# artpixls/ART

Measured on AMD Instinct MI355X. Metric: megapixels/sec end-to-end (AMaZE+FTblockDN+tone), 45 MP Bayer, higher is better.
Workload: dtype f32; 1 GPU; AMaZE + getImage/matrix + ImProcFunctions::denoise (chroma noise-curve map, FTblockDN wavelet shrinkage luma 40 / chroma 15 / gamma 1.7 + DCT detail recovery 50) + exposure 0.3 EV + tone curve STD, 8192x5464 Bayer RGGB fp32, 1 frame per GPU per step (BASELINE configs[2]); frame=8192x5464, lanes_per_gpu=1, parallelism=frame-per-gpu x1, completion_records=1, completion_via=single process

## Files before the change

art_amd/csrc/api_internal.h:

```cpp
#pragma once
#include <hip/hip_runtime.h>
#include <dlfcn.h>
#include <cmath>
#include <cstdio>
#include <cstdarg>
#include <cstring>
#include <new>
#include <string>
#include <thread>
#include <vector>
#include <algorithm>

#include "../../include/artgpu.h"
#include "kernels.h"
#include "dehaze.h"
#include "textureboost.h"
#include "colorcorrection.h"
#include "smoothing.h"
#include "toneequalizer.h"
#include "filmsim.h"
#include "masks.h"
#include "sharpen.h"

struct artgpu_ctx {
    int device = 0;
    hipStream_t stream = nullptr;
    hipStream_t aux = nullptr;
    hipEvent_t aux_ev[2] = {nullptr, nullptr};
    hipStream_t dn_stream[1] = {nullptr};
    hipEvent_t dn_ev[2] = {nullptr, nullptr};
    const float *gam_tab = nullptr; float gam_key[6] = {};
    struct Shared {
        int opt_sharpen_fused = 1;
        int opt_te_group_thread = 0;
        int opt_te_fuse_upsample = 1;
        int opt_lut_lds = 1;
        int opt_dn_streams = 0;
        int opt_dn_fused = 1;
        int opt_dn_detail_plain = 0;
        int opt_dn_mad_fold = 1;
        int opt_dn_mad_fold_grid = 0;
        int opt_dn_debug_stall = -1;
        long opt_dn_wait_ms = 0;
        int opt_io_direct = -1;
        int opt_cu_reserve = 0;
        int opt_amaze_path = 0;
        int opt_amaze_split = 0;
        long opt_amaze_zero_mask = 0x81f0;
        int opt_amaze_zero_frame = 16;
        int opt_amaze_poison = -1;
        int opt_roctx = 0;
        int opt_amaze_overlap = 1;
        int opt_amaze_grid = 0;
        int opt_rcd_rows = 8;
        int curve_tail_kind = ARTGPU_CURVE_TAIL_HOST;
        double curve_tail_y = 1.0;
        artgpu::ParamCurve curve_tail_pc = {};
        artgpu_progress_fn progress_fn = nullptr;
        void *progress_user = nullptr;
        const artgpu_mask_params *pipe_lc = nullptr, *pipe_tb = nullptr;
        int pipe_nlc = 0, pipe_ntb = 0;
        const artgpu_color_correction_region *pipe_cc = nullptr;
        const artgpu_mask_params *pipe_cc_masks = nullptr;
        int pipe_ncc = 0;
        const artgpu_smoothing_region *pipe_sm = nullptr;
        const artgpu_mask_params *pipe_sm_masks = nullptr;
        int pipe_nsm = 0;
        int pipe_te_on = 0;
        artgpu_tone_equalizer_params pipe_te = {};
        const artgpu_clut *pipe_fs = nullptr;
        artgpu_film_simulation_params pipe_fs_par = {};
        int pipe_fs_after = 0;
    } shared;
    float *sh_host = nullptr;
    hipEvent_t sh_ev = nullptr;
    struct PipeMasks { std::vector<artgpu_mask_params> m; std::vector<std::vector<double>> curves; std::vector<artgpu_plane> areas; } pipe_lc_own, pipe_tb_own;
    template <typename Region> struct PipeRegions { std::vector<Region> regs; std::vector<artgpu_plane> planes; PipeMasks masks; };
    PipeRegions<artgpu_color_correction_region> pipe_cc_own;
    PipeRegions<artgpu_smoothing_region> pipe_sm_own;
    artgpu_clut *pipe_fs_own = nullptr;
    std::string err;
    int *fs_diag = nullptr;
    long long batch_px = 0;
    const int *dn_fold_flags = nullptr; int dn_fold_ranges[8][2] = {}; int dn_fold_nranges = 0;
    int dn_form = -1, dn_form_streak = 0;
    float *arena = nullptr;
    size_t arena_bytes = 0;
    static constexpr int NSTAGE = 8;
    float *stage[NSTAGE] = {};
    size_t stage_bytes[NSTAGE] = {};
    static constexpr int NPOOL = 96;
    float *pool[NPOOL] = {};
// ... 222 lines not shown
```

art_amd/csrc/artgpu_api.hip:

```cpp
#include "api_internal.h"

using namespace artgpu;
using namespace artgpu::api;

namespace {

int const_table_dev(artgpu_ctx *ctx, int slot, size_t nfloats, void (*fill)(float *), const char *what, float **out)
{
    const bool fresh = ctx->pool[slot] == nullptr;
    const int rc = pool_get(ctx, slot, nfloats * 4, out);
    if (rc || !fresh) return rc;
    std::vector<float> host(nfloats);
    fill(host.data());
    hipError_t e = hipMemcpyAsync(*out, host.data(), nfloats * 4, hipMemcpyHostToDevice, ctx->stream);
    if (e == hipSuccess) e = hipStreamSynchronize(ctx->stream);
    if (e != hipSuccess) {
        (void)hipFree(ctx->pool[slot]); ctx->pool[slot] = nullptr; ctx->pool_bytes[slot] = 0;
        *out = nullptr;
        return fail(ctx, ARTGPU_EHIP, "upload of the %s failed: %s", what, hipGetErrorString(e));
    }
    return ARTGPU_OK;
}

void build_lab_tabs(float *host)
// ... 312 lines not shown
    HIPCHK(ctx, hipSetDevice(ctx->device));
    hipEvent_t ev = nullptr;
    if (hipEventCreateWithFlags(&ev, hipEventDisableTiming) == hipSuccess) {
        if (hipEventRecord(ev, ctx->stream) == hipSuccess) (void)hipStreamWaitEvent(next, ev, 0);
        (void)hipEventDestroy(ev);
    }
    (void)hipGetLastError();
    ctx->stream = next;
    return ARTGPU_OK;
}

int artgpu_synchronize(artgpu_ctx *ctx)
{
    if (!ctx) return ARTGPU_EINVAL;
    HIPCHK(ctx, hipSetDevice(ctx->device));
    HIPCHK(ctx, hipStreamSynchronize(ctx->stream));
    return check_async_faults(ctx);
}

int artgpu_set_curve_tail(artgpu_ctx *ctx, int kind, double y_last)
{
    if (!ctx) return ARTGPU_EINVAL;
    if (kind < ARTGPU_CURVE_TAIL_LUT || kind > ARTGPU_CURVE_TAIL_HOST) return fail(ctx, ARTGPU_EINVAL, "set_curve_tail: kind %d (a parametric curve: artgpu_set_curve_tail_parametric)", kind);
    ctx->shared.curve_tail_kind = kind;
    ctx->shared.curve_tail_y = y_last;
    return ARTGPU_OK;
}

int artgpu_set_curve_tail_parametric(artgpu_ctx *ctx, const double *p, int np)
{
    if (!ctx) return ARTGPU_EINVAL;
    if (!p || (np != 8 && np != 9)) return fail(ctx, ARTGPU_EINVAL, "set_curve_tail_parametric: 8 or 9 parameters (p[0] = DCT_Parametric)");
    if (p[4] == 0.0 && p[5] == 0.0 && p[6] == 0.0 && p[7] == 0.0) return fail(ctx, ARTGPU_EINVAL, "set_curve_tail_parametric: an identity curve has no Curve object (ARTGPU_CURVE_TAIL_LUT)");
    pc_init(ctx->shared.curve_tail_pc, p, np);
    ctx->shared.curve_tail_kind = ARTGPU_CURVE_TAIL_PARAMETRIC;
    return ARTGPU_OK;
}

int artgpu_get_option(artgpu_ctx *ctx, const char *name, long *value)
{
    if (!ctx || !name || !value) return ARTGPU_EINVAL;
    const std::string n(name);
    if (n.rfind("amaze_counter", 0) == 0 && n.size() == 14 && n[13] >= '0' && n[13] <= '7') {
        if (!ctx->amz_lists || ctx->amz_nstream <= 0) { *value = 0; return ARTGPU_OK; }
        HIPCHK(ctx, hipSetDevice(ctx->device));
        HIPCHK(ctx, hipStreamSynchronize(ctx->stream));
        const size_t nfixed = (((size_t)ctx->amz_nstream + (1 + ctx->amz_narena) + (1 + ctx->amz_narena + ctx->amz_nstream) + 3) / 4) * 4;
        int v = 0;
        HIPCHK(ctx, hipMemcpy(&v, reinterpret_cast<int *>(ctx->amz_lists) + nfixed + 4 + 2 * (size_t)ctx->amz_nstream + (n[13] - '0'), sizeof(int), hipMemcpyDeviceToHost));
        *value = v;
        return ARTGPU_OK;
    }
    if (n == "dn_mad_fold") { *value = ctx->shared.opt_dn_mad_fold; return ARTGPU_OK; }
    if (n == "cu_reserve") { *value = ctx->shared.opt_cu_reserve; return ARTGPU_OK; }
    if (n == "io_direct") { *value = ctx->shared.opt_io_direct; return ARTGPU_OK; }
    if (n == "te_group_thread") { *value = ctx->shared.opt_te_group_thread; return ARTGPU_OK; }
    if (n == "te_fuse_upsample") { *value = ctx->shared.opt_te_fuse_upsample; return ARTGPU_OK; }
    if (n.rfind("dn_mad_bits", 0) == 0 && n.size() > 11) {
        const int k = std::atoi(n.c_str() + 11);
        if (k < 0 || k > 95 || !ctx->dn_fold_flags) return fail(ctx, ARTGPU_EINVAL, "get_option: %s: word 0 .. 95 of a context that has denoised", name);
        HIPCHK(ctx, hipSetDevice(ctx->device));
        HIPCHK(ctx, hipStreamSynchronize(ctx->stream));
        int v = 0;
        HIPCHK(ctx, hipMemcpy(&v, ctx->dn_fold_flags - 96 + k, sizeof v, hipMemcpyDeviceToHost));
        *value = v;
        return ARTGPU_OK;
    }
    if (n == "dn_mad_fold_settled" || n == "dn_mad_fold_fallback") {
        HIPCHK(ctx, hipSetDevice(ctx->device));
        HIPCHK(ctx, hipStreamSynchronize(ctx->stream));
        int flags[96] = {};
        if (ctx->dn_fold_nranges) HIPCHK(ctx, hipMemcpy(flags, ctx->dn_fold_flags, sizeof flags, hipMemcpyDeviceToHost));
        const int want = n == "dn_mad_fold_settled" ? 1 : 2;
        long cnt = 0;
        for (int r = 0; r < ctx->dn_fold_nranges; ++r)
            for (int k = 0; k < ctx->dn_fold_ranges[r][1]; ++k) cnt += flags[ctx->dn_fold_ranges[r][0] + k] == want;
        *value = cnt;
        return ARTGPU_OK;
    }
    return fail(ctx, ARTGPU_EINVAL, "get_option: unknown option '%s'", name);
}

int artgpu_set_option(artgpu_ctx *ctx, const char *name, long value)
{
    if (!ctx || !name) return ARTGPU_EINVAL;
    const std::string n(name);
    if (n == "amaze_path") { if (value < 0 || value > 1) return fail(ctx, ARTGPU_EINVAL, "amaze_path: 0 or 1"); ctx->shared.opt_amaze_path = (int)value; }
    else if (n == "amaze_split") ctx->shared.opt_amaze_split = value != 0;
    else if (n == "amaze_overlap") ctx->shared.opt_amaze_overlap = value != 0;
    else if (n == "amaze_grid") { if (value < 0) return fail(ctx, ARTGPU_EINVAL, "amaze_grid: >= 0"); ctx->shared.opt_amaze_grid = (int)value; }
    else if (n == "amaze_zero_mask") ctx->shared.opt_amaze_zero_mask = value;
    else if (n == "amaze_zero_frame") ctx->shared.opt_amaze_zero_frame = (int)value;
    else if (n == "amaze_poison") ctx->shared.opt_amaze_poison = (int)value;
    else if (n == "roctx") ctx->shared.opt_roctx = value != 0;
    else if (n == "dn_streams") ctx->shared.opt_dn_streams = value != 0;
    else if (n == "dn_fused") ctx->shared.opt_dn_fused = (int)value;
    else if (n == "dn_mad_fold") ctx->shared.opt_dn_mad_fold = value != 0;
    else if (n == "dn_mad_fold_grid") { if (value < 0 || value > 65536) return fail(ctx, ARTGPU_EINVAL, "dn_mad_fold_grid: 0 (default) .. 65536 workgroups"); ctx->shared.opt_dn_mad_fold_grid = (int)value; }
    else if (n == "dn_detail_plain") { if (value < 0 || value > 3) return fail(ctx, ARTGPU_EINVAL, "dn_detail_plain: 0 .. 3"); ctx->shared.opt_dn_detail_plain = (int)value; }
    else if (n == "dn_debug_stall") ctx->shared.opt_dn_debug_stall = (int)value;
    else if (n == "dn_wait_ms") ctx->shared.opt_dn_wait_ms = value < 0 ? 0 : value;
    else if (n == "lut_lds") ctx->shared.opt_lut_lds = value != 0;
    else if (n == "te_group_thread") ctx->shared.opt_te_group_thread = value != 0;
    else if (n == "te_fuse_upsample") ctx->shared.opt_te_fuse_upsample = value != 0;
    else if (n == "sharpen_fused") ctx->shared.opt_sharpen_fused = value != 0;
    else if (n == "cu_reserve") { if (value < 0 || value > 4096) return fail(ctx, ARTGPU_EINVAL, "cu_reserve: 0 .. 4096"); ctx->shared.opt_cu_reserve = (int)value; }
    else if (n == "io_direct") { if (value < -1 || value > 4096) return fail(ctx, ARTGPU_EINVAL, "io_direct: -1 (automatic), 0 .. 4096 workgroups"); ctx->shared.opt_io_direct = (int)value; }
    else if (n == "rcd_rows") { if (value != 4 && value != 8) return fail(ctx, ARTGPU_EINVAL, "rcd_rows: 4 or 8"); ctx->shared.opt_rcd_rows = (int)value; }
    else return fail(ctx, ARTGPU_EINVAL, "set_option: unknown option '%s'", name);
    return ARTGPU_OK;
}

int artgpu_set_progress_callback(artgpu_ctx *ctx, artgpu_progress_fn fn, void *user)
{
    if (!ctx) return ARTGPU_EINVAL;
    ctx->shared.progress_fn = fn;
    ctx->shared.progress_user = user;
    return ARTGPU_OK;
}

int artgpu_enable_timing(artgpu_ctx *ctx, int enable)
{
    if (!ctx) return ARTGPU_EINVAL;
    ctx->timing = enable != 0;
    return ARTGPU_OK;
}

int artgpu_get_timings(const artgpu_ctx *ctx, artgpu_timings *out)
{
    if (!ctx || !out) return ARTGPU_EINVAL;
    *out = ctx->last;
    return ARTGPU_OK;
}

size_t artgpu_scratch_bytes(const artgpu_ctx *ctx)
{
    if (!ctx) return 0;
    size_t s = ctx->arena_bytes;
    for (int k = 0; k < artgpu_ctx::NSTAGE; ++k) s += ctx->stage_bytes[k];
    s += ctx->lut_bytes;
    for (int k = 0; k < artgpu_ctx::NPOOL; ++k) s += ctx->pool_bytes[k];
    return s;
}

int artgpu_trim_scratch(artgpu_ctx *ctx)
{
    if (!ctx) return ARTGPU_EINVAL;
    HIPCHK(ctx, hipSetDevice(ctx->device));
    HIPCHK(ctx, hipStreamSynchronize(ctx->stream));
    if (ctx->aux) HIPCHK(ctx, hipStreamSynchronize(ctx->aux));
    if (ctx->dn_stream[0]) HIPCHK(ctx, hipStreamSynchronize(ctx->dn_stream[0]));
    if (ctx->amz_side) HIPCHK(ctx, hipStreamSynchronize(ctx->amz_side));
// ... 349 lines not shown

}

namespace {

struct DnFusion {
    float pre_scale, post_scale;
    GetImageFuse gi;
    int exp_on;
    float exp_scale, exp_black;
    int tail_on;
    float tail_scale, tail_black;
    int ccalc_nonneg;
};

void build_dct_tabs(float *host)
{
    float *tm_in = host, *tm_out = tm_in + 4096, *ct = tm_out + 4096, *ctt = ct + 4096;
    const float epsilon = 0.001f / (64 * 64);
    const int border = 4;
    for (int i = 0; i < 64; ++i) {
        const float i1 = std::abs((i > 32 ? i - 64 + 1 : i));
        const float vmask = (i1 < border ? (float)0 + (std::sin((M_PI * i1) / (2 * border)) * std::sin((M_PI * i1) / (2 * border))) : 1.0f);
        const float vmask2 = (i1 < 2 * border ? (std::sin((M_PI * i1) / (2 * border)) * std::sin((M_PI * i1) / (2 * border))) : 1.0f);
        for (int j = 0; j < 64; ++j) {
            const float j1 = std::abs((j > 32 ? j - 64 + 1 : j));
            const double sj = std::sin((M_PI * j1) / (2 * border));
            tm_in[i * 64 + j] = (vmask * (j1 < border ? sj * sj : 1.0f)) + epsilon;
            tm_out[i * 64 + j] = (vmask2 * (j1 < 2 * border ? sj * sj : 1.0f)) + epsilon;
            ct[i * 64 + j] = (float)std::cos(M_PI * (j + 0.5) * i / 64.0);
            ctt[j * 64 + i] = ct[i * 64 + j];
        }
    }
}

struct DnPlan {
    int w, h, w2, h2;
    size_t n, n2;
    bool lab_mode, do_detail, useNoiseCCurve;
    float noisevarL;
    bool denoiseLuminance;
    float gam, gamthresh, gamslope, igam, igamthresh, igamslope, gain;
    float realred, realblue, noisevarab_r, noisevarab_b, maxNoiseVarab;
    bool aggressive, autoch;
    int levwav, nsub;
    bool too_small;
    int rad[10], maxrad;
    bool fork;
    bool mad_fold;
    int fold_g0, fold_g1;
    bool fused, merged, merged_mad;
    bool two_chroma;
    int detail_plain;
    long long wait_ticks;
    int stall_band, stall_strip;
};

DnPlan dn_plan(int w, int h, const artgpu_denoise_params *p, double scale, double expcomp, uint32_t flags, bool want_resid, bool has_ccalc,
               int opt_dn_streams, int opt_dn_fused, int opt_dn_detail_plain, long opt_dn_wait_ms, int opt_dn_debug_stall, int opt_dn_mad_fold, int opt_dn_mad_fold_grid)
{
    DnPlan pl = {};
    const int w2 = (w + 1) / 2, h2 = (h + 1) / 2;
    pl.w = w; pl.h = h; pl.w2 = w2; pl.h2 = h2; pl.n = (size_t)w * h; pl.n2 = (size_t)w2 * h2;
    pl.lab_mode = p->color_space == 1;
    pl.do_detail = !(flags & ARTGPU_DN_SKIP_DETAIL_RECOVERY);
    pl.useNoiseCCurve = has_ccalc;
    pl.detail_plain = opt_dn_detail_plain == 1 ? 3 : opt_dn_detail_plain == 2 ? 1 : opt_dn_detail_plain == 3 ? 2 : 0;
    pl.wait_ticks = (long long)opt_dn_wait_ms * 100000LL;
    pl.stall_band = opt_dn_debug_stall < 0 ? -1 : opt_dn_debug_stall >> 16;
    pl.stall_strip = opt_dn_debug_stall < 0 ? -1 : opt_dn_debug_stall & 0xffff;

    const float noiseluma = (float)p->luminance;
    const double nl_t = (noiseluma / 125.0) * (1.0 + noiseluma / 25.0);
    const float noisevarL = (float)(nl_t * nl_t);
    const bool denoiseLuminance = noisevarL > 0.00001f;
    const float gam = (float)p->gamma;
    const float gamthresh = 0.001f;
    const float gamslope = (float)(std::exp(std::log((double)gamthresh) / gam) / gamthresh);
    pl.noisevarL = noisevarL; pl.denoiseLuminance = denoiseLuminance;
    pl.gam = gam; pl.gamthresh = gamthresh; pl.gamslope = gamslope;
    pl.igam = 1.f / gam; pl.igamthresh = gamthresh * gamslope; pl.igamslope = 1.f / gamslope;
    pl.gain = std::pow(2.0f, float(expcomp));
    const float interm_med = (float)p->chrominance / 10.0;
    float intermred = p->chrominance_red_green > 0. ? (p->chrominance_red_green / 10.) : (float)p->chrominance_red_green / 7.0;
    float intermblue = p->chrominance_blue_yellow > 0. ? (p->chrominance_blue_yellow / 10.) : (float)p->chrominance_blue_yellow / 7.0;
    float realred = interm_med + intermred;
    if (realred <= 0.f) realred = 0.001f;
    float realblue = interm_med + intermblue;
    if (realblue <= 0.f) realblue = 0.001f;
    const float noisevarab_r = realred * realred, noisevarab_b = realblue * realblue;
    pl.realred = realred; pl.realblue = realblue; pl.noisevarab_r = noisevarab_r; pl.noisevarab_b = noisevarab_b;
    pl.maxNoiseVarab = noisevarab_b > noisevarab_r ? noisevarab_b : noisevarab_r;
    int levwav = 5;
    const float maxreal = realred > realblue ? realred : realblue;
    if (maxreal < 8.f) levwav = 5; else if (maxreal < 10.f) levwav = 6; else if (maxreal < 15.f) levwav = 7; else levwav = 8;
    const bool aggressive = p->aggressive != 0;
    if (aggressive) levwav += 2;
    if (levwav > 8) levwav = 8;
    { const int t = int(levwav - std::ceil(std::log(scale))); levwav = t > 5 ? t : 5; }
    const int minsizetile = w < h ? w : h;
    int maxlev2 = 8;
    if (minsizetile < 256) maxlev2 = 7;
    if (minsizetile < 128) maxlev2 = 6;
    if (minsizetile < 64) maxlev2 = 5;
    if (minsizetile < 32) maxlev2 = 4;
    if (minsizetile < 16) maxlev2 = 3;
    levwav = levwav < maxlev2 ? levwav : maxlev2;
    const int nsub = 3 * levwav;
    const bool autoch = p->chrominance_method == 1;
    pl.aggressive = aggressive; pl.autoch = autoch; pl.levwav = levwav; pl.nsub = nsub;
    pl.too_small = (w2 < h2 ? w2 : h2) < 2 * wavelet_skip(levwav - 1) || w < 8 || h < 8;
    if (pl.too_small) return pl;

    pl.fork = opt_dn_streams != 0 && pl.do_detail && denoiseLuminance;

    pl.maxrad = 1;
    for (int l = 0; l < levwav; ++l) { const int r = int((l + 2) / scale); pl.rad[l] = r > 1 ? r : 1; pl.maxrad = pl.rad[l] > pl.maxrad ? pl.rad[l] : pl.maxrad; }
    pl.fused = opt_dn_fused != 0 && shrink_blur_supported(w2, h2, pl.rad, 0, nsub);
    pl.merged = pl.fused && opt_dn_fused != 2 && !aggressive && !want_resid && denoiseLuminance && levwav <= 5 &&
                (autoch || (noisevarab_r > 0.001f && noisevarab_b > 0.001f));
// ... 245 lines not shown
    if (!pl.denoiseLuminance) return ARTGPU_OK;
    int rc2;
    const int nsub = pl.nsub, nsubL = 3 * (pl.levwav < 5 ? pl.levwav : 5);
    const size_t n2 = pl.n2;
    const DevDecomp &Ld = b.Ld;
    float *sf = b.sfc[0], *tmp = b.tmpc[0];
    BlurArgs bl = blur0();
    ShrinkArgs sa = {};
    sa.coef = Ld.bands; sa.sfave = sf; sa.n = n2; sa.madL = b.mad; sa.noisevar = nullptr; sa.noisevar_const = pl.noisevarL;
    DevDecomp Lrec = Ld;
    if (pl.merged) Lrec.bands = b.Lbands2;
    for (int rep = pl.aggressive ? 0 : 1; rep < 2 && !pl.merged; ++rep) {
        if (pl.fused) {
            float *dstb = b.Lbands2 ? b.Lbands2 : Ld.bands;
            if ((rc2 = fused_pass(false, Lrec.bands, dstb, nullptr, b.mad, nullptr, 0, nsubL, pl.noisevarL, 0.f))) return rc2;
            Lrec.bands = dstb;
        } else {
            HIPCHK(ctx, launch_shrink_sf(sa, nsubL, false, sL));
            bl.src = sf; bl.dst = tmp;
            HIPCHK(ctx, launch_hblur(bl, nsubL, sL));
            bl.src = tmp; bl.sfave = sf; bl.coef = Ld.bands;
            HIPCHK(ctx, launch_vblur_combine(bl, nsubL, sL));
        }
    }
    if (Lrec.bands != Ld.bands && nsubL < nsub)
        HIPCHK(ctx, hipMemcpyAsync(Lrec.bands + (size_t)nsubL * n2, Ld.bands + (size_t)nsubL * n2, (size_t)(nsub - nsubL) * n2 * 4, hipMemcpyDeviceToDevice, sL));
    if (pl.do_detail) {
        if ((rc2 = pool_get(ctx, P_LIN, pl.n * 4, &Lout))) return rc2;
    }
    Lrec.cur = Ld.cur;
    if ((rc2 = reconstruct_dev(ctx, Lrec, Lout, sL))) return rc2;
    return pl.do_detail ? detail_recovery(sd) : ARTGPU_OK;
}

int DnRun::detail_recovery(hipStream_t sd)
{
    const int w = pl.w, h = pl.h;
    int rc2;
    DetailArgs da = {};
    da.w = w; da.h = h;
    da.numblox_W = (int)std::ceil(((float)w) / 25) + 2;
    da.numblox_H = (int)std::ceil(((float)h) / 25) + 2;
    const float params_Ldetail = std::min(float(p->luminance_detail), 99.9f);
    auto compute_detail = [](float dd) -> float { const float t = static_cast<float>((100. - dd) * (100. - dd) + 50. * (100. - dd)) * 64 * 0.5f; return t * t; };
    da.detail_hi = compute_detail(params_Ldetail);
    da.detail_lo = compute_detail(0.f);
    { const int br = int(3 / scale); da.blur_rad = br > 1 ? br : 1; }
    float *dtab;
    if ((rc2 = const_table_dev(ctx, P_DCTTAB, 4 * 4096, build_dct_tabs, "DCT tables", &dtab))) return rc2;
    if ((rc2 = pool_get(ctx, P_BLOCKS, (size_t)da.numblox_W * da.numblox_H * 4096 * 4, &da.blocks))) return rc2;
    da.tm_in = dtab; da.tm_out = dtab + 4096; da.costab = dtab + 2 * 4096; da.costab_t = dtab + 3 * 4096;
    da.L = Lout; da.Lin = b.L;
    da.plain = pl.detail_plain;
    if (p->luminance_detail_threshold > 0) {
        float *dmask;
        if ((rc2 = pool_get(ctx, P_DMASK, pl.n * 4, &dmask))) return rc2;
        const float amount = std::max(0.f, std::min(float(p->luminance_detail_threshold) / 100.f, 1.f));
        float *dm_scratch = b.tmpc[0];
        if (!dm_scratch && (rc2 = pool_get(ctx, P_TMP, ((size_t)w * h + 2 * (size_t)(w / 4) * (h / 4)) * 4, &dm_scratch))) return rc2;
        if ((rc2 = detail_mask_dev(ctx, Lout, (size_t)w, dmask, w, h, 65535.f, 25.f, 10000.f, amount, (float)(25.f / scale), dm_scratch))) return rc2;
        da.mask = dmask; da.params_Ldetail = params_Ldetail;
    }
    if (sd != sL) {
        HIPCHK(ctx, hipEventRecord(ctx->dn_ev[0], sL));
        HIPCHK(ctx, hipStreamWaitEvent(sd, ctx->dn_ev[0], 0));
    }
    HIPCHK(ctx, launch_detail_blocks(da, sd));
    HIPCHK(ctx, launch_detail_gather(da, sd));
    if (sd != sL) HIPCHK(ctx, hipEventRecord(ctx->dn_ev[1], sd));
    return ARTGPU_OK;
}

int DnRun::merged_pass()
{
    const int nsub = pl.nsub;
    FusedShrinkArgs fa = fused_args(pl.noisevarL);
    fa.coef = b.Ld.bands; fa.coef_out = b.Lbands2; fa.coefC = b.Cdd[0].bands; fa.coefL = b.Ld.bands;
    fa.madL = b.mad; fa.madab = pl.merged_mad ? b.mad + nsub : b.mad + 32; fa.mad_ch_stride = nsub;
    fa.noisevar_ab[0] = noisevar_abc[0]; fa.noisevar_ab[1] = noisevar_abc[1];
    fa.level0 = 0; fa.nsub = 3 * nsub; fa.nL = nsub; fa.nsub_ch = nsub;
    HIPCHK(ctx, launch_shrink_blur(fa, b.fused_scratch, sL));
    return ARTGPU_OK;
}

int rgb_denoise_args_ok(artgpu_ctx *ctx, const artgpu_denoise_params *p, const float *iws, double scale)
{
    if (p->color_space != 0 && p->color_space != 1) return fail(ctx, ARTGPU_EINVAL, "rgb_denoise: color_space must be 0 (RGB) or 1 (LAB)");
    if (p->color_space == 1 && !iws) return fail(ctx, ARTGPU_EINVAL, "rgb_denoise: LAB mode needs the inverse working-space matrix");
    if (p->chrominance_method != 0 && p->chrominance_method != 1) return fail(ctx, ARTGPU_EINVAL, "rgb_denoise: chrominance_method must be 0 (MANUAL) or 1 (AUTOMATIC)");
    if (!(scale >= 1.0)) return fail(ctx, ARTGPU_EINVAL, "rgb_denoise: scale must be >= 1");
    return ARTGPU_OK;
}

int rgb_denoise_dev(artgpu_ctx *ctx, const DevRGB &d, const artgpu_denoise_params *p, const float ws[9], const float *iws,
                    double expcomp, double scale, const artgpu_plane *ccalc, uint32_t flags, float *nresi, float *highresi, const DnFusion &fu)
{
    const int w = d.w, h = d.h;
    if (w > 32767 || h > 32767) return fail(ctx, ARTGPU_EUNSUPPORTED, "rgb_denoise: the reference holds the size in short (FTblockDN.cc:1779)");
    if (p->luminance == 0 && p->chrominance == 0 && !ccalc) return ARTGPU_OK;
    const DnPlan pl = dn_plan(w, h, p, scale, expcomp, flags, nresi || highresi, ccalc != nullptr,
                              ctx->shared.opt_dn_streams, ctx->shared.opt_dn_fused, ctx->shared.opt_dn_detail_plain, ctx->shared.opt_dn_wait_ms, ctx->shared.opt_dn_debug_stall, ctx->shared.opt_dn_mad_fold, ctx->shared.opt_dn_mad_fold_grid);
    if (pl.too_small) return fail(ctx, ARTGPU_EUNSUPPORTED, "rgb_denoise: %dx%d too small for %d wavelet levels on the device path", w, h, pl.levwav);
    DnBuffers b;
    int rc = dn_buffers(ctx, pl, ccalc, &b);
    if (rc) return rc;
    if (pl.fork && !ctx->dn_stream[0]) {
        HIPCHK(ctx, hipStreamCreateWithFlags(&ctx->dn_stream[0], hipStreamNonBlocking));
        for (int k = 0; k < 2; ++k) HIPCHK(ctx, hipEventCreateWithFlags(&ctx->dn_ev[k], hipEventDisableTiming));
    }
    hipStream_t sL = ctx->stream;

    {
        const float key[6] = {pl.gam, pl.gamthresh, pl.gamslope, pl.igam, pl.igamthresh, pl.igamslope};
        if (ctx->gam_tab != b.gamlut || std::memcmp(ctx->gam_key, key, sizeof key) != 0) {
            ctx->gam_tab = nullptr;
            HIPCHK(ctx, launch_gamma_lut(b.gamlut, pl.gam, pl.gamthresh, pl.gamslope, 65535.f, 65535.f, sL));
            HIPCHK(ctx, launch_gamma_lut(b.gamlut + 65536, pl.igam, pl.igamthresh, pl.igamslope, 65535.f, 65535.f, sL));
            std::memcpy(ctx->gam_key, key, sizeof key);
            ctx->gam_tab = b.gamlut;
        }
    }

    DnPixArgs px = {};
    for (int k = 0; k < 3; ++k) { px.rgb[k] = d.p[k]; px.ws1[k] = ws[3 + k]; }
    px.stride = d.stride; px.L = b.L; px.A = b.A; px.B = b.B; px.w = w; px.h = h;
    px.gain = pl.gain; px.newGain = 1.f / pl.gain;
    px.gam = pl.gam; px.gamthresh = pl.gamthresh; px.gamslope = pl.gamslope; px.igam = pl.igam; px.igamthresh = pl.igamthresh; px.igamslope = pl.igamslope;
    px.gamcurve = b.gamlut; px.igamcurve = b.gamlut + 65536;
    px.pre_scale = fu.pre_scale; px.post_scale = fu.post_scale; px.no_lds_lut = !ctx->shared.opt_lut_lds; px.cu_reserve = cu_reserve_of(ctx);
    px.gi = fu.gi; px.exp_on = fu.exp_on; px.exp_scale = fu.exp_scale; px.exp_black = fu.exp_black;
    px.igam_lds_lo = 8000;
    if (pl.lab_mode) {
        float *tabs;
        if ((rc = lab_tabs_dev(ctx, &tabs))) return rc;
        px.lab_mode = 1;
        px.cachef = tabs; px.cachefy = tabs + 65536; px.dn_gamma = tabs + 2 * 65536; px.dn_igamma = tabs + 3 * 65536;
        for (int k = 0; k < 9; ++k) { px.wpi[k] = ws[k]; px.iws[k] = iws[k]; }
    }
    px.realred = pl.realred; px.realblue = pl.realblue; px.qhighFactor = pl.aggressive ? 1.f / static_cast<float>(0.9) : 1.0f;
    HIPCHK(ctx, launch_rgb2yuv(px, sL));

    ctx->dn_fold_nranges = 0; ctx->dn_fold_flags = b.fold_flags;
    if ((rc = decompose_dev(ctx, b.Ld, b.L, sL))) return rc;
    DnRun run = {ctx, pl, b, fu, p, scale, nresi, highresi, sL, {0.f, 0.f}, 0.f, 0.f, b.L};
    if (!pl.merged_mad && (rc = run.mad_decomposed(b.Ld.bands, pl.nsub, reinterpret_cast<int *>(b.histo_fc[0]), b.mad))) return rc;

    if (pl.merged) {
        if ((rc = run.chroma_front(0)) || (rc = run.chroma_front(1))) return rc;
        if (pl.merged_mad && (rc = run.mad_decomposed(b.Ld.bands, 3 * pl.nsub, reinterpret_cast<int *>(b.histo_fc[0]), b.mad))) return rc;
        if ((rc = run.merged_pass())) return rc;
        SideStreamJoin dn_join;
        if (pl.fork) dn_join.arm(ctx->dn_stream[0]);
        if ((rc = run.luma(pl.fork ? ctx->dn_stream[0] : sL))) return rc;
        if ((rc = run.chroma_back(0)) || (rc = run.chroma_back(1))) return rc;
// ... 2209 lines not shown
```

art_amd/csrc/detail.hip:

```cpp
#include <hip/hip_runtime.h>
#include <type_traits>
#include "devmath.h"
#include "devsleef.h"
#include "dct64.h"
#include "kernels.h"

namespace artgpu {

namespace {
constexpr int TS = 64, OFF = 25, BLKRAD = 1;
constexpr int XR = 4;
constexpr int NXCD = 8;
__device__ __forceinline__ int reflect(int v, int n)
{
    if (v < 0) return -v < n - 1 ? -v : n - 1;
    if (v >= n) return 2 * n - 2 - v > 0 ? 2 * n - 2 - v : 0;
    return v;
}
}

#ifdef DETAIL_PHASE_MARKS
#define DETAIL_PHASE(name) asm volatile("; detail-phase " name)
#else
#define DETAIL_PHASE(name)
// ... 253 lines not shown
                Ldetail = v ? ld : Ldetail;
                totwt = v ? tw : totwt;
            }
        a.L[t] = Lold + Ldetail / totwt;
    }
#else
    for (long long t = blockIdx.x * (long long)blockDim.x + threadIdx.x; t < n; t += (long long)gridDim.x * blockDim.x) {
        const int y = (int)(t / a.w), x = (int)(t - (long long)y * a.w);
        const int vb0 = max(0, y / OFF + BLKRAD - 2), vb1 = min(a.numblox_H - 1, y / OFF + BLKRAD);
        const int hb0 = max(0, x / OFF + BLKRAD - 2), hb1 = min(a.numblox_W - 1, x / OFF + BLKRAD);
        float Ldetail = 0.f, totwt = 0.f;
        for (int vblk = vb0; vblk <= vb1; ++vblk) {
            const int i = y - (vblk - BLKRAD) * OFF;
            if (i < 0 || i >= TS) continue;
            for (int hblk = hb0; hblk <= hb1; ++hblk) {
                const int j = x - (hblk - BLKRAD) * OFF;
                if (j < 0 || j >= TS) continue;
                const float tmo = s_out[i * TS + j];
                Ldetail += tmo * a.blocks[((size_t)vblk * a.numblox_W + hblk) * TS * TS + i * TS + j] * DCTnorm;
                totwt += s_in[i * TS + j] * tmo;
            }
        }
        a.L[t] += Ldetail / totwt;
    }
#endif
}

__global__ void __launch_bounds__(1024) detail_gather_rows_kernel(DetailArgs a)
{
    __shared__ float s_in[TS * TS], s_out[TS * TS], s_tw[OFF * OFF];
    for (int k = threadIdx.x; k < TS * TS; k += 1024) { s_in[k] = a.tm_in[k]; s_out[k] = a.tm_out[k]; }
    __syncthreads();
    constexpr int NEAR = TS - 2 * OFF;
    for (int k = threadIdx.x; k < OFF * OFF; k += 1024) {
        const int ry = k / OFF, rx = k - ry * OFF;
        float totwt = 0.f;
#pragma unroll
        for (int s_ = 0; s_ < 3; ++s_)
#pragma unroll
            for (int t_ = 0; t_ < 3; ++t_) {
                const bool v = (s_ > 0 || ry < NEAR) && (t_ > 0 || rx < NEAR);
                const int m = v ? (ry + 2 * OFF - OFF * s_) * TS + rx + 2 * OFF - OFF * t_ : 0;
                const float tw = totwt + s_in[m] * s_out[m];
                totwt = v ? tw : totwt;
            }
        s_tw[k] = totwt;
    }
    __syncthreads();
    const float DCTnorm = 1.0f / (4 * TS * TS);
    const int wave = __builtin_amdgcn_readfirstlane(threadIdx.x >> 6), lane = threadIdx.x & 63;
    const int ncx = (a.w + 63) / 64, ncy = (a.h + OFF - 1) / OFF;
    const int nunits = ncx * ncy;
    const size_t brow = (size_t)a.numblox_W * TS * TS;
    for (int u = wave * gridDim.x + blockIdx.x; u < nunits; u += 16 * gridDim.x) {
        const int yc = __builtin_amdgcn_readfirstlane(u / ncx), cx = u - yc * ncx;
        const int x = cx * 64 + lane;
        const bool xin = x < a.w;
        const int xx = xin ? x : a.w - 1;
        const int xc = xx / OFF, rx = xx - xc * OFF;
        const bool h0 = xc > 0 && rx < NEAR;
        int jh[3];
        unsigned co[3];
#pragma unroll
        for (int t_ = 0; t_ < 3; ++t_) {
            const bool hs = t_ > 0 || h0;
            jh[t_] = hs ? rx + 2 * OFF - OFF * t_ : rx;
            co[t_] = (unsigned)((hs ? xc - 1 + t_ : xc + 1) * (TS * TS) + jh[t_]) * 4u;
        }
        const int rows = min(OFF, a.h - yc * OFF);
        const int rows0 = yc > 0 ? min(rows, NEAR) : 0;
        const unsigned lo = (unsigned)(xx - cx * 64) * 4u;
        char *Lrow = (char *)(a.L + ((size_t)yc * OFF * a.w + (size_t)cx * 64));
        const char *b0 = (const char *)(a.blocks + ((size_t)(yc > 0 ? yc - 1 : 0) * brow + 2 * OFF * TS));
        const char *b1 = (const char *)(a.blocks + ((size_t)yc * brow + OFF * TS));
        const char *b2 = (const char *)(a.blocks + (size_t)(yc + 1) * brow);
        const bool whole = yc > 0 && xc > 0;
        auto row = [&](const int ry, auto above) {
            constexpr bool V0 = decltype(above)::value;
            constexpr int S0 = V0 ? 0 : 1;
            const size_t ro = (size_t)ry * TS * 4;
            const char *bs[3] = {b0 + ro, b1 + ro, b2 + ro};
            float blk[9], tmo[9];
#pragma unroll
            for (int s_ = S0; s_ < 3; ++s_)
#pragma unroll
                for (int t_ = 0; t_ < 3; ++t_) {
                    blk[3 * s_ + t_] = *(const float *)(bs[s_] + co[t_]);
                    tmo[3 * s_ + t_] = s_out[(ry + 2 * OFF - OFF * s_) * TS + jh[t_]];
                }
            const float Lold = *(const float *)(Lrow + (size_t)ry * a.w * 4 + lo);
            float Ldetail = 0.f;
#pragma unroll
            for (int s_ = S0; s_ < 3; ++s_)
#pragma unroll
                for (int t_ = 0; t_ < 3; ++t_) {
                    const float ld = Ldetail + tmo[3 * s_ + t_] * blk[3 * s_ + t_] * DCTnorm;
                    Ldetail = (t_ > 0 || h0) ? ld : Ldetail;
                }
            float totwt;
            if (whole) totwt = s_tw[ry * OFF + rx];
            else {
                totwt = 0.f;
#pragma unroll
                for (int s_ = S0; s_ < 3; ++s_)
#pragma unroll
                    for (int t_ = 0; t_ < 3; ++t_) {
                        const int m = (ry + 2 * OFF - OFF * s_) * TS + jh[t_];
                        const float tw = totwt + s_in[m] * s_out[m];
                        totwt = (t_ > 0 || h0) ? tw : totwt;
                    }
            }
            if (xin) *(float *)(Lrow + (size_t)ry * a.w * 4 + lo) = Lold + Ldetail / totwt;
        };
        for (int ry = 0; ry < rows0; ++ry) row(ry, std::true_type());
        for (int ry = rows0; ry < rows; ++ry) row(ry, std::false_type());
    }
}

hipError_t launch_detail_blocks(const DetailArgs &a_, hipStream_t s)
{
    DetailArgs a = a_;
    if (a.plain & 1) {
        const dim3 grid(NXCD * ((a.numblox_W + NXCD - 1) / NXCD) * a.numblox_H);
        switch (a.blur_rad) {
        case 1: hipLaunchKernelGGL(detail_blocks_kernel<1>, grid, dim3(64), 0, s, a); break;
        case 2: hipLaunchKernelGGL(detail_blocks_kernel<2>, grid, dim3(64), 0, s, a); break;
        case 3: hipLaunchKernelGGL(detail_blocks_kernel<3>, grid, dim3(64), 0, s, a); break;
        default: return hipErrorInvalidValue;
        }
        return hipGetLastError();
    }
    a.inside32 = (long long)a.w * a.h <= (1LL << 30);
    const dim3 grid(NXCD * ((a.numblox_W - 1 + NXCD - 1) / NXCD) * (a.numblox_H - 1));
    switch (a.blur_rad) {
    case 1: hipLaunchKernelGGL(detail_blocks_trim_kernel<1>, grid, dim3(64), 0, s, a); break;
    case 2: hipLaunchKernelGGL(detail_blocks_trim_kernel<2>, grid, dim3(64), 0, s, a); break;
    case 3: hipLaunchKernelGGL(detail_blocks_trim_kernel<3>, grid, dim3(64), 0, s, a); break;
    default: return hipErrorInvalidValue;
    }
    return hipGetLastError();
}
hipError_t launch_detail_gather(const DetailArgs &a, hipStream_t s)
{
    int dev = 0, cus = 256;
    if (hipGetDevice(&dev) == hipSuccess) (void)hipDeviceGetAttribute(&cus, hipDeviceAttributeMultiprocessorCount, dev);
    const long long cap = 2LL * cus;
    const long long units = ((long long)a.w + 63) / 64 * (((long long)a.h + OFF - 1) / OFF);
    if (!(a.plain & 2) && (long long)a.numblox_W * TS * TS * 4 < (1LL << 32) && units + 16 * cap < (1LL << 31)) {
        const long long g = (units + 15) / 16;
        hipLaunchKernelGGL(detail_gather_rows_kernel, dim3((int)(g < cap ? g : cap)), dim3(1024), 0, s, a);
        return hipGetLastError();
    }
    const long long n = (long long)a.w * a.h;
    const long long g = (n + 1023) / 1024;
    hipLaunchKernelGGL(detail_gather_kernel, dim3((int)(g < cap ? g : cap)), dim3(1024), 0, s, a);
    return hipGetLastError();
}

}
```

art_amd/csrc/kernels.h:

```cpp
#pragma once
#include <hip/hip_runtime.h>
#include "paramcurve.h"
#include <vector>
#include <stddef.h>
#include <stdint.h>
#include <mutex>
#include <set>
#include <utility>

inline hipError_t dyn_lds_once(const void *fn, int bytes)
{
    static std::mutex m;
    static std::set<std::pair<const void *, int>> done;
    int dev = 0;
    hipError_t e = hipGetDevice(&dev);
    if (e != hipSuccess) return e;
    std::lock_guard<std::mutex> lk(m);
    if (done.count({fn, dev})) return hipSuccess;
    e = hipFuncSetAttribute(fn, hipFuncAttributeMaxDynamicSharedMemorySize, bytes);
    if (e == hipSuccess) done.insert({fn, dev});
    return e;
}

inline bool device_block_fits(int lds_bytes, int threads)
// ... 413 lines not shown
constexpr int MAD_SCRATCH_INTS_PER_BAND = 8 + 1024 + 4096 + 8;
hipError_t launch_mad(const float *bands, size_t n, int nsub, int *histo, float *out, hipStream_t s);
hipError_t launch_mad_fold(const float *bands, size_t n, int nsub, int nsub_ch, const int *cnt, int *histo, float *out, int *flags, hipStream_t s);
hipError_t launch_shrink_sf(const ShrinkArgs &a, int nsub, bool ab, hipStream_t s);
hipError_t launch_hblur(const BlurArgs &a, int nsub, hipStream_t s);
hipError_t launch_vblur_combine(const BlurArgs &a, int nsub, hipStream_t s);
struct FusedShrinkArgs {
    const float *coef;
    float *coef_out;
    float *coefC;
    const float *coefL;
    size_t n;
    int w, h;
    const float *madL;
    const float *madab;
    const float *noisevar;
    int noisevar_nonneg;
    float noisevar_const;
    float noisevar_scale;
    float noisevar_ab[2];
    int useNoiseCCurve;
    int rad[10];
    int level0;
    int nsub;
    int nL;
    int nsub_ch;
    int mad_ch_stride;
    int nstrips;
    float *hand;
    int wpad;
    int *progress;
    int *ticket;
    int *diag;
    long long wait_ticks;
    int stall_band, stall_strip;
    long long *prof;
};
bool shrink_blur_supported(int w, int h, const int *rad, int level0, int nsub);
size_t shrink_blur_scratch_floats(int w, int h, int nsub, int maxr);
hipError_t launch_shrink_blur(FusedShrinkArgs a, float *scratch, hipStream_t s);

struct DetailArgs {
    float *L;
    const float *Lin;
    const float *tm_in, *tm_out;
    const float *costab, *costab_t;
    float *blocks;
    int w, h, numblox_W, numblox_H;
    float detail_hi, detail_lo;
    int blur_rad;
    const float *mask;
    float params_Ldetail;
    int plain;
    int inside32;
};
hipError_t launch_detail_blocks(const DetailArgs &a, hipStream_t s);
hipError_t launch_detail_gather(const DetailArgs &a, hipStream_t s);

struct GuidedArgs {
    float *rgb[3];
    size_t stride;
    int W, H;
    int w, h;
    float *in[3];
    float *guide;
    float *chan[3];
    float *low[8];
    double ws1[3];
    float epsilon;
    int nch;
    float *q; size_t q_stride;
};
hipError_t launch_gf_prepare(const GuidedArgs &a, hipStream_t s);
hipError_t launch_gf_subsample(const GuidedArgs &a, hipStream_t s);
hipError_t launch_gf_ab(const GuidedArgs &a, hipStream_t s);
hipError_t launch_gf_finish(const GuidedArgs &a, hipStream_t s);
hipError_t launch_gf_finish_plain(const GuidedArgs &a, hipStream_t s);

struct MaskArgs {
    const float *src; size_t src_stride;
    float *L2, *m2;
    float *mask;
    int W, H, w4, h4;
    float scaling, threshold, ceiling, factor;
};
struct GaussArgs {
    float *img, *tmp;
    double *tmp64;
    int W, H;
    double B, b[3], M[9];
    float Bf, bf[3], Mf[9];
};
struct NlmArgs {
    float *img; size_t img_stride;
    float *src;
    float *mask;
    float *SW;
    float *explut;
    int W, H, WW, HH, border, search_radius, patch_radius, ntiles_x, ntiles_y;
    float factor, h2;
};
hipError_t launch_detail_mask(const MaskArgs &a, hipStream_t s);
hipError_t launch_gaussian(const GaussArgs &a, hipStream_t s);
hipError_t launch_gaussian3(float *img, float *tmp, int W, int H, float c0, float c1, hipStream_t s);
hipError_t launch_nlm(const NlmArgs &a, hipStream_t s);
bool nlm_group_supported(const NlmArgs &a);
// ... 65 lines not shown
```

Before: 4642 MP/s.

## Group detail-gather wavefronts on adjacent units with periodic workgroup barriers

The detail-recovery gather kernel now gives the 16 wavefronts of a workgroup consecutive column-strip units instead of units strided across the grid. Every five rows the wavefronts meet at a workgroup barrier, so neighbouring strips move through the block buffer together and share cache lines. Idle wavefronts run the loop with zero rows so they still reach each barrier. The old strided mapping is kept behind a new plain-bit value, and a new option overrides the grid cap; the cost is barrier stalls inside the row loop.

```diff
diff --git a/art_amd/csrc/api_internal.h b/art_amd/csrc/api_internal.h
--- a/art_amd/csrc/api_internal.h
+++ b/art_amd/csrc/api_internal.h
@@ -38,6 +38,7 @@
         int opt_dn_streams = 0;
         int opt_dn_fused = 1;
         int opt_dn_detail_plain = 0;
+        int opt_dn_detail_gather_grid = 0;
         int opt_dn_mad_fold = 1;
         int opt_dn_mad_fold_grid = 0;
         int opt_dn_debug_stall = -1;
diff --git a/art_amd/csrc/artgpu_api.hip b/art_amd/csrc/artgpu_api.hip
--- a/art_amd/csrc/artgpu_api.hip
+++ b/art_amd/csrc/artgpu_api.hip
@@ -388,6 +388,8 @@
         return ARTGPU_OK;
     }
     if (n == "dn_mad_fold") { *value = ctx->shared.opt_dn_mad_fold; return ARTGPU_OK; }
+    if (n == "dn_detail_plain") { *value = ctx->shared.opt_dn_detail_plain; return ARTGPU_OK; }
+    if (n == "dn_detail_gather_grid") { *value = ctx->shared.opt_dn_detail_gather_grid; return ARTGPU_OK; }
     if (n == "cu_reserve") { *value = ctx->shared.opt_cu_reserve; return ARTGPU_OK; }
     if (n == "io_direct") { *value = ctx->shared.opt_io_direct; return ARTGPU_OK; }
     if (n == "te_group_thread") { *value = ctx->shared.opt_te_group_thread; return ARTGPU_OK; }
@@ -433,7 +435,8 @@
     else if (n == "dn_fused") ctx->shared.opt_dn_fused = (int)value;
     else if (n == "dn_mad_fold") ctx->shared.opt_dn_mad_fold = value != 0;
     else if (n == "dn_mad_fold_grid") { if (value < 0 || value > 65536) return fail(ctx, ARTGPU_EINVAL, "dn_mad_fold_grid: 0 (default) .. 65536 workgroups"); ctx->shared.opt_dn_mad_fold_grid = (int)value; }
-    else if (n == "dn_detail_plain") { if (value < 0 || value > 3) return fail(ctx, ARTGPU_EINVAL, "dn_detail_plain: 0 .. 3"); ctx->shared.opt_dn_detail_plain = (int)value; }
+    else if (n == "dn_detail_plain") { if (value < 0 || value > 4) return fail(ctx, ARTGPU_EINVAL, "dn_detail_plain: 0 .. 4"); ctx->shared.opt_dn_detail_plain = (int)value; }
+    else if (n == "dn_detail_gather_grid") { if (value < 0 || value > 65536) return fail(ctx, ARTGPU_EINVAL, "dn_detail_gather_grid: 0 (default) .. 65536 workgroups"); ctx->shared.opt_dn_detail_gather_grid = (int)value; }
     else if (n == "dn_debug_stall") ctx->shared.opt_dn_debug_stall = (int)value;
     else if (n == "dn_wait_ms") ctx->shared.opt_dn_wait_ms = value < 0 ? 0 : value;
     else if (n == "lut_lds") ctx->shared.opt_lut_lds = value != 0;
@@ -889,12 +892,13 @@
     bool fused, merged, merged_mad;
     bool two_chroma;
     int detail_plain;
+    int detail_gather_grid;
     long long wait_ticks;
     int stall_band, stall_strip;
 };
 
 DnPlan dn_plan(int w, int h, const artgpu_denoise_params *p, double scale, double expcomp, uint32_t flags, bool want_resid, bool has_ccalc,
-               int opt_dn_streams, int opt_dn_fused, int opt_dn_detail_plain, long opt_dn_wait_ms, int opt_dn_debug_stall, int opt_dn_mad_fold, int opt_dn_mad_fold_grid)
+               int opt_dn_streams, int opt_dn_fused, int opt_dn_detail_plain, long opt_dn_wait_ms, int opt_dn_debug_stall, int opt_dn_mad_fold, int opt_dn_mad_fold_grid, int opt_dn_detail_gather_grid)
 {
     DnPlan pl = {};
     const int w2 = (w + 1) / 2, h2 = (h + 1) / 2;
@@ -902,7 +906,8 @@
     pl.lab_mode = p->color_space == 1;
     pl.do_detail = !(flags & ARTGPU_DN_SKIP_DETAIL_RECOVERY);
     pl.useNoiseCCurve = has_ccalc;
-    pl.detail_plain = opt_dn_detail_plain == 1 ? 3 : opt_dn_detail_plain == 2 ? 1 : opt_dn_detail_plain == 3 ? 2 : 0;
+    pl.detail_plain = opt_dn_detail_plain == 1 ? 3 : opt_dn_detail_plain == 2 ? 1 : opt_dn_detail_plain == 3 ? 2 : opt_dn_detail_plain == 4 ? 4 : 0;
+    pl.detail_gather_grid = opt_dn_detail_gather_grid;
     pl.wait_ticks = (long long)opt_dn_wait_ms * 100000LL;
     pl.stall_band = opt_dn_debug_stall < 0 ? -1 : opt_dn_debug_stall >> 16;
     pl.stall_strip = opt_dn_debug_stall < 0 ? -1 : opt_dn_debug_stall & 0xffff;
@@ -1254,6 +1259,7 @@
     da.tm_in = dtab; da.tm_out = dtab + 4096; da.costab = dtab + 2 * 4096; da.costab_t = dtab + 3 * 4096;
     da.L = Lout; da.Lin = b.L;
     da.plain = pl.detail_plain;
+    da.gather_grid = pl.detail_gather_grid;
     if (p->luminance_detail_threshold > 0) {
         float *dmask;
         if ((rc2 = pool_get(ctx, P_DMASK, pl.n * 4, &dmask))) return rc2;
@@ -1301,7 +1307,7 @@
     if (w > 32767 || h > 32767) return fail(ctx, ARTGPU_EUNSUPPORTED, "rgb_denoise: the reference holds the size in short (FTblockDN.cc:1779)");
     if (p->luminance == 0 && p->chrominance == 0 && !ccalc) return ARTGPU_OK;
     const DnPlan pl = dn_plan(w, h, p, scale, expcomp, flags, nresi || highresi, ccalc != nullptr,
-                              ctx->shared.opt_dn_streams, ctx->shared.opt_dn_fused, ctx->shared.opt_dn_detail_plain, ctx->shared.opt_dn_wait_ms, ctx->shared.opt_dn_debug_stall, ctx->shared.opt_dn_mad_fold, ctx->shared.opt_dn_mad_fold_grid);
+                              ctx->shared.opt_dn_streams, ctx->shared.opt_dn_fused, ctx->shared.opt_dn_detail_plain, ctx->shared.opt_dn_wait_ms, ctx->shared.opt_dn_debug_stall, ctx->shared.opt_dn_mad_fold, ctx->shared.opt_dn_mad_fold_grid, ctx->shared.opt_dn_detail_gather_grid);
     if (pl.too_small) return fail(ctx, ARTGPU_EUNSUPPORTED, "rgb_denoise: %dx%d too small for %d wavelet levels on the device path", w, h, pl.levwav);
     DnBuffers b;
     int rc = dn_buffers(ctx, pl, ccalc, &b);
diff --git a/art_amd/csrc/detail.hip b/art_amd/csrc/detail.hip
--- a/art_amd/csrc/detail.hip
+++ b/art_amd/csrc/detail.hip
@@ -329,7 +329,13 @@
     const int ncx = (a.w + 63) / 64, ncy = (a.h + OFF - 1) / OFF;
     const int nunits = ncx * ncy;
     const size_t brow = (size_t)a.numblox_W * TS * TS;
-    for (int u = wave * gridDim.x + blockIdx.x; u < nunits; u += 16 * gridDim.x) {
+    constexpr int SYNC_ROWS = 5;
+    const bool grouped = !(a.plain & 4);
+    const int u0 = grouped ? 16 * (int)blockIdx.x + wave : wave * (int)gridDim.x + (int)blockIdx.x;
+    const int per = 16 * (int)gridDim.x, rounds = (nunits + per - 1) / per;
+    for (int k = 0; k < rounds; ++k) {
+        const bool live = u0 + k * per < nunits;
+        const int u = live ? u0 + k * per : 0;
         const int yc = __builtin_amdgcn_readfirstlane(u / ncx), cx = u - yc * ncx;
         const int x = cx * 64 + lane;
         const bool xin = x < a.w;
@@ -344,7 +350,7 @@
             jh[t_] = hs ? rx + 2 * OFF - OFF * t_ : rx;
             co[t_] = (unsigned)((hs ? xc - 1 + t_ : xc + 1) * (TS * TS) + jh[t_]) * 4u;
         }
-        const int rows = min(OFF, a.h - yc * OFF);
+        const int rows = live ? min(OFF, a.h - yc * OFF) : 0;
         const int rows0 = yc > 0 ? min(rows, NEAR) : 0;
         const unsigned lo = (unsigned)(xx - cx * 64) * 4u;
         char *Lrow = (char *)(a.L + ((size_t)yc * OFF * a.w + (size_t)cx * 64));
@@ -389,8 +395,11 @@
             }
             if (xin) *(float *)(Lrow + (size_t)ry * a.w * 4 + lo) = Lold + Ldetail / totwt;
         };
-        for (int ry = 0; ry < rows0; ++ry) row(ry, std::true_type());
-        for (int ry = rows0; ry < rows; ++ry) row(ry, std::false_type());
+        for (int ry = 0; ry < OFF; ++ry) {
+            if (grouped && ry % SYNC_ROWS == 0) __syncthreads();
+            if (ry < rows0) row(ry, std::true_type());
+            else if (ry < rows) row(ry, std::false_type());
+        }
     }
 }
 
@@ -421,7 +430,8 @@
 {
     int dev = 0, cus = 256;
     if (hipGetDevice(&dev) == hipSuccess) (void)hipDeviceGetAttribute(&cus, hipDeviceAttributeMultiprocessorCount, dev);
-    const long long cap = 2LL * cus;
+    long long cap = 2LL * cus;
+    if (a.gather_grid > 0) cap = a.gather_grid;
     const long long units = ((long long)a.w + 63) / 64 * (((long long)a.h + OFF - 1) / OFF);
     if (!(a.plain & 2) && (long long)a.numblox_W * TS * TS * 4 < (1LL << 32) && units + 16 * cap < (1LL << 31)) {
         const long long g = (units + 15) / 16;
diff --git a/art_amd/csrc/kernels.h b/art_amd/csrc/kernels.h
--- a/art_amd/csrc/kernels.h
+++ b/art_amd/csrc/kernels.h
@@ -489,6 +489,7 @@
     const float *mask;
     float params_Ldetail;
     int plain;
+    int gather_grid;
     int inside32;
 };
 hipError_t launch_detail_blocks(const DetailArgs &a, hipStream_t s);
```

After: 4636 MP/s, median of 2. About the same (-0.1%).
